# nfrasser/lasgun

Measured on NVIDIA B200. Metric: Mrays/s (primary+shadow), higher is better.
Workload: dtype f64

## Files before the change

### lasgun_b200/csrc/lgb_kernels.cu

```cuda
#include <math_constants.h>

#include <algorithm>

#include "lgb_math.cuh"

#ifndef LGB_SMEM_STACK
#define LGB_SMEM_STACK 0
#endif
#ifndef LGB_SMEM_TOP
#define LGB_SMEM_TOP 0
#endif
#define LGB_STK(i) ((i) * stride)
#ifndef LGB_WALK_PREFETCH
#define LGB_WALK_PREFETCH 0
#endif
#ifndef LGB_CP_STAGE
#define LGB_CP_STAGE 0
#endif
#ifndef LGB_WAVE_STREAM
#define LGB_WAVE_STREAM 1
#endif
#ifndef LGB_WALK_SPLIT
#define LGB_WALK_SPLIT 1
#endif
#ifndef LGB_WALK_SPLIT_SHADOW
#define LGB_WALK_SPLIT_SHADOW 0
#endif

namespace lgb {

#if LGB_WAVE_STREAM
template <class T> __device__ __forceinline__ void wst(T* p, T v) { __stcs(p, v); }
template <class T> __device__ __forceinline__ T wld(const T* p) { return __ldcs(p); }
#else
template <class T> __device__ __forceinline__ void wst(T* p, T v) { *p = v; }
template <class T> __device__ __forceinline__ T wld(const T* p) { return *p; }
#endif

struct RayF {
    float ox, oy, oz;
    float ix, iy, iz;
    float nx, ny, nz;
    float dx, dy, dz;
    float inv_dd, inv_len;
    float sx, sy, sz;
    float err;
    int kz;
    unsigned oct;
};

__device__ __forceinline__ float clamp_idir(float d) {
    const float v = 1.0f / d;
    return fabsf(v) > 1e30f ? copysignf(1e30f, v) : v;
}

__device__ __forceinline__ RayF make_rayf(const Ray64& r, float err_abs) {
    RayF f;
    f.ox = (float)r.o.x; f.oy = (float)r.o.y; f.oz = (float)r.o.z;
    f.dx = (float)r.d.x; f.dy = (float)r.d.y; f.dz = (float)r.d.z;
    f.oct = (signbit(r.d.x) ? 1u : 0u) | (signbit(r.d.y) ? 2u : 0u) | (signbit(r.d.z) ? 4u : 0u);
    f.ix = clamp_idir(f.dx); f.iy = clamp_idir(f.dy); f.iz = clamp_idir(f.dz);
    f.nx = -f.ox * f.ix; f.ny = -f.oy * f.iy; f.nz = -f.oz * f.iz;
    float dd = f.dx * f.dx + f.dy * f.dy + f.dz * f.dz;
    f.inv_dd = 1.0f / dd;
    f.inv_len = rsqrtf(dd);
    f.err = (dd > 1e-24f && dd < 1e24f) ? err_abs : CUDART_INF_F;
    f.kz = max_dimension_abs(r.d);
    const int kx = (f.kz + 1) % 3, ky = (kx + 1) % 3;
    float fdz = f.kz == 0 ? f.dx : (f.kz == 1 ? f.dy : f.dz);
    float fdx = kx == 0 ? f.dx : (kx == 1 ? f.dy : f.dz);
    float fdy = ky == 0 ? f.dx : (ky == 1 ? f.dy : f.dz);
    f.sz = 1.0f / fdz;
    f.sx = -fdx * f.sz;
    f.sy = -fdy * f.sz;
    return f;
}

__device__ __forceinline__ bool slab2(float lx, float ly, float lz, float hx, float hy, float hz, const RayF& f, float tbest_up, float& tnear_out) {
    float t1x = __fmaf_rn(lx, f.ix, f.nx), t2x = __fmaf_rn(hx, f.ix, f.nx);
    float t1y = __fmaf_rn(ly, f.iy, f.ny), t2y = __fmaf_rn(hy, f.iy, f.ny);
    float t1z = __fmaf_rn(lz, f.iz, f.nz), t2z = __fmaf_rn(hz, f.iz, f.nz);
    float tnear = fmaxf(fmaxf(fminf(t1x, t2x), fminf(t1y, t2y)), fminf(t1z, t2z));
    float tfar = fminf(fminf(fmaxf(t1x, t2x), fmaxf(t1y, t2y)), fmaxf(t1z, t2z));
    tnear_out = tnear;
    return tnear <= tfar * (1.0f + 9.5367431640625e-7f) && tfar > 0.0f && tnear <= tbest_up;
}
template <int OCT>
__device__ __forceinline__ bool slab_oct(float lx, float ly, float lz, float hx, float hy, float hz, const RayF& f, float tbest_up, float& tnear_out) {
    const float tnx = __fmaf_rn((OCT & 1) ? hx : lx, f.ix, f.nx), tfx = __fmaf_rn((OCT & 1) ? lx : hx, f.ix, f.nx);
    const float tny = __fmaf_rn((OCT & 2) ? hy : ly, f.iy, f.ny), tfy = __fmaf_rn((OCT & 2) ? ly : hy, f.iy, f.ny);
    const float tnz = __fmaf_rn((OCT & 4) ? hz : lz, f.iz, f.nz), tfz = __fmaf_rn((OCT & 4) ? lz : hz, f.iz, f.nz);
    const float tnear = fmaxf(fmaxf(tnx, tny), tnz);
    const float tfar = fminf(fminf(tfx, tfy), tfz) * (1.0f + 9.5367431640625e-7f);
    tnear_out = tnear;
    return fmaxf(tnear, 0.0f) <= fminf(tfar, tbest_up);
}
__device__ __forceinline__ float inflate_up(double t) { return __double2float_ru(t) * (1.0f + 9.5367431640625e-7f); }

struct Hit { double t; uint32_t ref; };

__device__ __forceinline__ DevCounters* ctr(const DevOut& O) {
    return reinterpret_cast<DevCounters*>(reinterpret_cast<char*>(O.counters) + (size_t)(1u + ((blockIdx.x + (threadIdx.x >> 5) * 17u) & (kCtrStripes - 1u))) * kCtrStride);
}
struct LocalCounters { unsigned int node_tests, filter[3], exact[3]; };

__device__ __forceinline__ uint32_t canonical_id(const DevScene& S, uint32_t ref) {
    const uint32_t type = ref >> 30, idx = ref & 0x3FFFFFFFu;
    if (type == LGB_PRIM_SPHERE) return S.sph_id[idx];
    if (type == LGB_PRIM_CUBOID) return S.cub_id[idx];
// ... 165 lines not shown
            if (tc + half + slack < 0.0f) continue;
            if (STATS) lc.exact[0]++;
            const double2 c01 = __ldg(reinterpret_cast<const double2*>(S.sph64 + 4 * (size_t)idx));
            const double2 c23 = __ldg(reinterpret_cast<const double2*>(S.sph64 + 4 * (size_t)idx + 2));
            double t; bool inside;
            if (sphere_exact(d3(c01.x, c01.y, c23.x), c23.y, ray, t, inside)) {
                const uint32_t ref = LGB_PRIM_REF(LGB_PRIM_SPHERE, idx);
                if (ANYHIT) { if (t < tmax) { best.t = t; best.ref = ref; return true; } }
                else if (accepts<INST>(S, f, world, best, t, ref, T.tied)) { best.t = t; best.ref = ref; best_tf = __double2float_ru(t); best_up = inflate_up(t); }
            }
        }
    } else {
        for (uint32_t i = 0; i < count; i++) {
            const uint32_t idx = first + i;
            const float4 lo = __ldg(&S.cub32[2 * idx]), hi = __ldg(&S.cub32[2 * idx + 1]);
            if (STATS) lc.filter[1]++;
            float tn;
            if (!slab2(lo.x, lo.y, lo.z, hi.x, hi.y, hi.z, f, CUDART_INF_F, tn)) continue;
            if (STATS) lc.exact[1]++;
            double mn[3], mx[3];
#pragma unroll
            for (int k = 0; k < 3; k++) { mn[k] = __ldg(&S.cub64[6 * (size_t)idx + k]); mx[k] = __ldg(&S.cub64[6 * (size_t)idx + 3 + k]); }
            double t; int ua, va;
            if (cuboid_exact(mn, mx, ray, t, ua, va)) {
                const uint32_t ref = LGB_PRIM_REF(LGB_PRIM_CUBOID, idx);
                if (ANYHIT) { if (t < tmax) { best.t = t; best.ref = ref; return true; } }
                else if (accepts<INST>(S, f, world, best, t, ref, T.tied)) { best.t = t; best.ref = ref; best_tf = __double2float_ru(t); best_up = inflate_up(t); }
            }
        }
    }
    return false;
}

template <bool STATS>
__device__ __forceinline__ bool prim_filter_rec(const RayF& f, float best_tf, uint32_t type, const float4 q0, const float4 q1, const float4 q2, LocalCounters& lc) {
    if (type == LGB_PRIM_SPHERE) {
        const float4 s = q0;
        if (STATS) lc.filter[0]++;
        const float lx = s.x - f.ox, ly = s.y - f.oy, lz = s.z - f.oz;
        const float bq = lx * f.dx + ly * f.dy + lz * f.dz;
        const float tc = bq * f.inv_dd;
        const float wx = __fmaf_rn(-tc, f.dx, lx), wy = __fmaf_rn(-tc, f.dy, ly), wz = __fmaf_rn(-tc, f.dz, lz);
        const float perp2 = wx * wx + wy * wy + wz * wz;
        const float rr = s.w + 2.0f * f.err;
        if (perp2 > rr * rr * (1.0f + 1e-6f)) return false;
        const float half = rr * f.inv_len;
        const float slack = fabsf(tc) * 2e-6f + 2.0f * f.err * f.inv_len;
        if (tc - half - slack > best_tf) return false;
        if (tc + half + slack < 0.0f) return false;
        return true;
    }
    if (type == LGB_PRIM_TRIANGLE) {
        if (STATS) lc.filter[2]++;
        return f.kz == 0 ? tri_filter<0>(q0, q1, q2, f, best_tf) : f.kz == 1 ? tri_filter<1>(q0, q1, q2, f, best_tf) : tri_filter<2>(q0, q1, q2, f, best_tf);
    }
    if (STATS) lc.filter[1]++;
    float tn;
    return slab2(q0.x, q0.y, q0.z, q1.x, q1.y, q1.z, f, CUDART_INF_F, tn);
}
__device__ __forceinline__ void prim_record(const DevScene& S, uint32_t type, uint32_t idx, float4& q0, float4& q1, float4& q2) {
    if (type == LGB_PRIM_SPHERE) q0 = __ldg(&S.sph32[idx]);
    else if (type == LGB_PRIM_TRIANGLE) { const float4* tp = S.tri + 3 * (size_t)idx; q0 = __ldg(tp); q1 = __ldg(tp + 1); q2 = __ldg(tp + 2); }
    else { q0 = __ldg(&S.cub32[2 * idx]); q1 = __ldg(&S.cub32[2 * idx + 1]); }
}
template <bool STATS>
__device__ __forceinline__ bool prim_filter(const DevScene& S, const RayF& f, float best_tf, uint32_t type, uint32_t idx, LocalCounters& lc) {
    float4 q0, q1 = make_float4(0.f, 0.f, 0.f, 0.f), q2 = q1;
    prim_record(S, type, idx, q0, q1, q2);
    return prim_filter_rec<STATS>(f, best_tf, type, q0, q1, q2, lc);
}
template <bool ANYHIT, bool STATS>
__device__ __forceinline__ bool prim_exact(const DevScene& S, const Ray64& world, const Ray64& ray, const RayF& f, Trav& T, uint32_t type, uint32_t idx, double tmax,
                                           LocalCounters& lc) {
    Hit& best = T.best;
    double t; bool ok;
    if (type == LGB_PRIM_SPHERE) {
        if (STATS) lc.exact[0]++;
        const double2 c01 = __ldg(reinterpret_cast<const double2*>(S.sph64 + 4 * (size_t)idx));
        const double2 c23 = __ldg(reinterpret_cast<const double2*>(S.sph64 + 4 * (size_t)idx + 2));
        bool inside;
        ok = sphere_exact(d3(c01.x, c01.y, c23.x), c23.y, ray, t, inside);
    } else if (type == LGB_PRIM_TRIANGLE) {
        if (STATS) lc.exact[2]++;
        const float4* tp = S.tri + 3 * (size_t)idx;
        const float4 q0 = __ldg(tp), q1 = __ldg(tp + 1), q2 = __ldg(tp + 2);
        double b0, b1, b2;
        ok = triangle_exact(d3(q0.x, q0.y, q0.z), d3(q1.x, q1.y, q1.z), d3(q2.x, q2.y, q2.z), ray, t, b0, b1, b2);
    } else {
        if (STATS) lc.exact[1]++;
        double mn[3], mx[3];
#pragma unroll
        for (int k = 0; k < 3; k++) { mn[k] = __ldg(&S.cub64[6 * (size_t)idx + k]); mx[k] = __ldg(&S.cub64[6 * (size_t)idx + 3 + k]); }
        int ua, va;
        ok = cuboid_exact(mn, mx, ray, t, ua, va);
    }
    if (!ok) return false;
    const uint32_t ref = LGB_PRIM_REF(type, idx);
    if (ANYHIT) { if (t < tmax) { best.t = t; best.ref = ref; return true; } return false; }
    if (accepts<false>(S, f, world, best, t, ref, T.tied)) { best.t = t; best.ref = ref; T.best_tf = __double2float_ru(t); T.best_up = inflate_up(t); }
    return false;
}

constexpr uint32_t kInstLeaf = kLeafBit | ((uint32_t)LGB_PRIM_INSTANCE << 29);
constexpr uint32_t kExitMarker = kInstLeaf | (31u << 24);
template <bool ANYHIT, bool STATS, bool REFILL, bool INST>
__device__ __forceinline__ bool trav_run(const DevScene& S, const Ray64& world, Ray64& ray, RayF& f, Trav& T, uint32_t* stack, float* tstack, double tmax,
                                         LocalCounters& lc, int refill_below, unsigned octw, const float4* top = nullptr, const int stride = 1) {
    Hit& best = T.best;
    float& best_tf = T.best_tf; float& best_up = T.best_up;
    uint32_t& cur = T.cur; int& sp = T.sp;
    for (;;) {
        switch (INST ? f.oct : octw) {
        case 0: node_loop<0, STATS, (!ANYHIT && LGB_TSTACK)>(S, f, best_up, cur, sp, stack, tstack, lc, top, stride); break;
        case 1: node_loop<1, STATS, (!ANYHIT && LGB_TSTACK)>(S, f, best_up, cur, sp, stack, tstack, lc, top, stride); break;
        case 2: node_loop<2, STATS, (!ANYHIT && LGB_TSTACK)>(S, f, best_up, cur, sp, stack, tstack, lc, top, stride); break;
        case 3: node_loop<3, STATS, (!ANYHIT && LGB_TSTACK)>(S, f, best_up, cur, sp, stack, tstack, lc, top, stride); break;
        case 4: node_loop<4, STATS, (!ANYHIT && LGB_TSTACK)>(S, f, best_up, cur, sp, stack, tstack, lc, top, stride); break;
        case 5: node_loop<5, STATS, (!ANYHIT && LGB_TSTACK)>(S, f, best_up, cur, sp, stack, tstack, lc, top, stride); break;
        case 6: node_loop<6, STATS, (!ANYHIT && LGB_TSTACK)>(S, f, best_up, cur, sp, stack, tstack, lc, top, stride); break;
        case 7: node_loop<7, STATS, (!ANYHIT && LGB_TSTACK)>(S, f, best_up, cur, sp, stack, tstack, lc, top, stride); break;
        default: node_loop<8, STATS, (!ANYHIT && LGB_TSTACK)>(S, f, best_up, cur, sp, stack, tstack, lc, top, stride); break;
        }
        if (cur == kDone) return true;
        {
            const uint32_t type = (cur >> 29) & 3u, count = ((cur >> 24) & 31u) + 1u, first = cur & kLeafFirstMask;
            if (INST && type == LGB_PRIM_INSTANCE) {
                if (count == 32u) {
                    T.space = first;
                    ray = ray_to_space(S, first, world);
                    f = make_rayf(ray, S.spaces[first].err_abs);
                } else {
                    if (count > 1u) { if (!ANYHIT && LGB_TSTACK) tstack[LGB_STK(sp)] = -CUDART_INF_F; stack[LGB_STK(sp)] = kInstLeaf | ((count - 2u) << 24) | (first + 1u); sp++; }
                    if (!ANYHIT && LGB_TSTACK) tstack[LGB_STK(sp)] = -CUDART_INF_F;
// ... 903 lines not shown
__device__ __noinline__ void setup_generic_slot(const DevScene* Sg, double ox, double oy, double oz, double dx, double dy, double dz, double t, uint32_t ref,
                                                double* ps_out, uint32_t* gate_out) {
    const DevScene& S = *Sg;
    Ray64 ray; ray.o = d3(ox, oy, oz); ray.d = d3(dx, dy, dz);
    ShadePoint P; uint32_t id;
    shade_point<false, false>(S, ray, t, ref, P, id);
    ps_out[0] = P.ps.x; ps_out[1] = P.ps.y; ps_out[2] = P.ps.z;
    *gate_out = light_gates(S, ray, P.ps, P.ng, dot(P.wo, P.ng), false);
}
#ifndef LGB_CPRIMARY_THREADS
#define LGB_CPRIMARY_THREADS 128
#endif
#ifndef LGB_CPRIMARY_BLOCKS
#define LGB_CPRIMARY_BLOCKS (1280 / LGB_CPRIMARY_THREADS)
#endif
template <bool STATS, bool SETUP = false>
__global__ void __launch_bounds__(LGB_CPRIMARY_THREADS, LGB_CPRIMARY_BLOCKS) k_cprimary(DevScene S, DevCamera C, DevWork W, DevOut O, DevWave V) {
    const uint64_t total = W.n_pixels * W.spp;
    const uint64_t g = (uint64_t)blockIdx.x * blockDim.x + threadIdx.x;
    const unsigned lane = threadIdx.x & 31u;
    LocalCounters lc = {};
    unsigned int hits = 0, primary = 0;
    bool valid = false;
    uint32_t x = 0, y = 0, s = 0;
    if (g < total) {
        const uint32_t p = fdiv((uint32_t)g, W.fd_spp);
        s = (uint32_t)g - p * W.spp;
        if (!slot_to_pixel(W, p, x, y)) { wst(&V.hit_t[g], (double)(CUDART_INF)); wst(&V.hit_ref[g], (uint32_t)(kSlotUnused)); }
        else valid = true;
    }
    const size_t cell = (size_t)(y >> W.cg_shift) * W.cg_nx + (size_t)(x >> W.cg_shift);
    uint32_t b = 0, e = 0;
    if (valid) { b = __ldg(W.cg_start + cell); e = __ldg(W.cg_start + cell + 1); }
#if LGB_CP_STAGE
    constexpr uint32_t kStage = 32;
    __shared__ uint2 s_ent[LGB_CPRIMARY_THREADS / 32][kStage];
    __shared__ float4 s_rec[LGB_CPRIMARY_THREADS / 32][kStage][3];
    const unsigned wid = threadIdx.x >> 5;
    uint32_t ns = 0;
    {
        const unsigned vmask = __ballot_sync(0xFFFFFFFFu, valid);
        if (vmask) {
            const int lead = __ffs(vmask) - 1;
            const unsigned long long cell0 = __shfl_sync(0xFFFFFFFFu, (unsigned long long)cell, lead);
            const uint32_t b0 = __shfl_sync(0xFFFFFFFFu, b, lead), e0 = __shfl_sync(0xFFFFFFFFu, e, lead);
            if (__all_sync(0xFFFFFFFFu, !valid || (unsigned long long)cell == cell0)) {
                ns = min(e0 - b0, kStage);
                if (lane < ns) {
                    const uint2 r = __ldg(W.cg_entries + b0 + lane);
                    float4 q0, q1 = make_float4(0.f, 0.f, 0.f, 0.f), q2 = q1;
                    prim_record(S, r.x >> 30, r.x & 0x3FFFFFFFu, q0, q1, q2);
                    s_ent[wid][lane] = r;
                    s_rec[wid][lane][0] = q0; s_rec[wid][lane][1] = q1; s_rec[wid][lane][2] = q2;
                }
                __syncwarp();
            }
        }
    }
#endif
    if (valid) {
        {
            const Ray64 world = camera_ray(C, W, x, y, s);
            Ray64 ray; RayF f; Trav T;
            enter_root<false>(S, world, ray, f, T, CUDART_INF);
            primary++;
            const float to_t = f.inv_len * (1.0f - 2e-6f);
            const bool sorted = e - b <= kGridSortMax;
#if LGB_WALK_SPLIT
            const uint32_t e2 = e + W.cg_n_large;
            for (uint32_t i = b;;) {
                uint32_t cand = 0xFFFFFFFFu;
                while (i < e2) {
                    const bool in_cell = i < e;
#if LGB_CP_STAGE
                    const uint32_t k = i - b;
                    const bool staged = k < ns;
                    const uint2 r = staged ? s_ent[wid][k] : __ldg(in_cell ? W.cg_entries + i : W.cg_large + (i - e));
                    i++;
                    if (__uint_as_float(r.y) * to_t > T.best_up) { if (!in_cell) i = e2; else if (sorted) i = e; continue; }
                    const uint32_t type = r.x >> 30;
                    float4 q0, q1 = make_float4(0.f, 0.f, 0.f, 0.f), q2 = q1;
                    if (staged) { q0 = s_rec[wid][k][0]; if (type != LGB_PRIM_SPHERE) { q1 = s_rec[wid][k][1]; q2 = s_rec[wid][k][2]; } }
                    else prim_record(S, type, r.x & 0x3FFFFFFFu, q0, q1, q2);
                    if (prim_filter_rec<STATS>(f, T.best_tf, type, q0, q1, q2, lc)) { cand = r.x; break; }
#else
                    const uint2 r = __ldg(in_cell ? W.cg_entries + i : W.cg_large + (i - e));
                    i++;
                    if (__uint_as_float(r.y) * to_t > T.best_up) { if (!in_cell) i = e2; else if (sorted) i = e; continue; }
                    if (prim_filter<STATS>(S, f, T.best_tf, r.x >> 30, r.x & 0x3FFFFFFFu, lc)) { cand = r.x; break; }
#endif
                }
                if (cand == 0xFFFFFFFFu) break;
                prim_exact<false, STATS>(S, world, ray, f, T, cand >> 30, cand & 0x3FFFFFFFu, CUDART_INF, lc);
            }
#else
#if LGB_WALK_PREFETCH
            uint2 nxt = b < e ? __ldg(W.cg_entries + b) : make_uint2(0u, 0u);
            for (uint32_t i = b; i < e; i++) {
                const uint2 r = nxt;
                if (i + 1 < e) nxt = __ldg(W.cg_entries + i + 1);
#else
            for (uint32_t i = b; i < e; i++) {
                const uint2 r = __ldg(W.cg_entries + i);
#endif
                if (__uint_as_float(r.y) * to_t > T.best_up) { if (sorted) break; else continue; }
                leaf_prims<false, STATS, false>(S, world, ray, f, T, r.x >> 30, 1u, r.x & 0x3FFFFFFFu, CUDART_INF, lc);
            }
            for (uint32_t i = 0; i < W.cg_n_large; i++) {
                const uint2 r = __ldg(W.cg_large + i);
                if (__uint_as_float(r.y) * to_t > T.best_up) break;
                leaf_prims<false, STATS, false>(S, world, ray, f, T, r.x >> 30, 1u, r.x & 0x3FFFFFFFu, CUDART_INF, lc);
            }
#endif
            const bool hit = T.best.ref != LGB_MISS;
            wst(&V.hit_t[g], (double)(hit ? T.best.t : CUDART_INF)); wst(&V.hit_ref[g], (uint32_t)(T.best.ref));
            hits += hit ? 1u : 0u;
            if (T.tied) { const uint32_t k = atomicAdd(V.tie_count, 1u); if (k < V.tie_cap) V.tie_list[k] = (uint32_t)g; }
            if (SETUP && hit) {
                const uint32_t ref = T.best.ref; const double t = T.best.t;
                if (S.specular && (material_flags(S, ref) & kMatSpecular)) { wst(&V.occl[g], (uint32_t)(0)); wst(&V.gate[g], (uint32_t)(0)); }
                else {
                    LeanSurf Ls;
                    lean_surface<true>(S, world, t, ref, 0u, Ls);
                    if (Ls.flags & kSfGeneric) setup_generic_slot(S.self, world.o.x, world.o.y, world.o.z, world.d.x, world.d.y, world.d.z, t, ref, V.ps + 3 * g, V.gate + g);
                    else {
                        const D3 ng = (Ls.flags & kSfNgFlip) ? -Ls.n : Ls.n;
                        const D3 ps = world.o + world.d * t + ng * (2.220446049250313e-16 * 65536.0);
                        wst(&V.ps[3 * g + 0], ps.x); wst(&V.ps[3 * g + 1], ps.y); wst(&V.ps[3 * g + 2], ps.z);
                        wst(&V.gate[g], (uint32_t)(light_gates(S, world, ps, ng, 1.0, true)));
                    }
                    wst(&V.sflags[g], (unsigned char)((unsigned char)Ls.flags));
                    wst(&V.occl[g], (uint32_t)(0));
                }
            }
        }
    }
    if (O.counters) {
        const unsigned long long v0 = __popc(__ballot_sync(0xFFFFFFFFu, primary != 0)), v1 = __popc(__ballot_sync(0xFFFFFFFFu, hits != 0));
        if (lane == 0) { atomicAdd(&ctr(O)->primary_rays, v0); atomicAdd(&ctr(O)->primary_hits, v1); }
        if (STATS) {
            for (int k = 0; k < 3; k++) {
                unsigned long long a = warp_sum(lc.filter[k]), b = warp_sum(lc.exact[k]);
                if (lane == 0) { atomicAdd(&ctr(O)->filter[k], a); atomicAdd(&ctr(O)->exact[k], b); atomicAdd(&ctr(O)->p_filter[k], a); atomicAdd(&ctr(O)->p_exact[k], b); }
            }
        }
    }
// ... 264 lines not shown
            const double* Lp = S.lights + 9 * (size_t)light;
            Ray64 world;
            world.o = d3(V.ps[3 * (size_t)g], V.ps[3 * (size_t)g + 1], V.ps[3 * (size_t)g + 2]);
            world.d = d3(Lp[0], Lp[1], Lp[2]) - world.o;
            Ray64 ray; RayF f; Trav T;
            enter_root<false>(S, world, ray, f, T, 1.0);
            bool hit = false;
            for (uint32_t k = 0; k < n && !hit; k++) {
                const uint2 e = __ldg(&list_in[(size_t)k * W.n_pixels + p]);
                hit = leaf_prims<true, STATS, false>(S, world, ray, f, T, (e.x >> 29) & 3u, 1u, e.x & kLeafFirstMask, 1.0, lc);
            }
            if (hit) { atomicOr(&V.occl[g], 1u << light); occluded++; }
            *slot = kEntryDone;
        }
    }
    if (O.counters) {
        unsigned long long v = warp_sum(occluded);
        if (lane == 0 && v) atomicAdd(&ctr(O)->shadow_occluded, v);
        if (STATS) {
            for (int k = 0; k < 3; k++) {
                unsigned long long a = warp_sum(lc.filter[k]), b = warp_sum(lc.exact[k]);
                if (lane == 0) { atomicAdd(&ctr(O)->filter[k], a); atomicAdd(&ctr(O)->exact[k], b); }
            }
        }
    }
}

#ifndef LGB_GSHADOW_THREADS
#define LGB_GSHADOW_THREADS 64
#endif
#ifndef LGB_GSHADOW_MIN_BLOCKS
#define LGB_GSHADOW_MIN_BLOCKS (1536 / LGB_GSHADOW_THREADS)
#endif
template <bool STATS>
__device__ __forceinline__ bool grid_blocked(const DevScene& S, D3 o, uint32_t l, LocalCounters& lc) {
    Ray64 world;
    world.o = o;
    const double* Lp = S.lights + 9 * (size_t)l;
    world.d = d3(Lp[0], Lp[1], Lp[2]) - world.o;
    const double ax = fabs(world.d.x), ay = fabs(world.d.y), az = fabs(world.d.z);
    const int a = ax >= ay ? (ax >= az ? 0 : 2) : (ay >= az ? 1 : 2);
    const double da = -(a == 0 ? world.d.x : a == 1 ? world.d.y : world.d.z);
    const double db = -(a == 0 ? world.d.y : a == 1 ? world.d.z : world.d.x), dc = -(a == 0 ? world.d.z : a == 1 ? world.d.x : world.d.y);
    if (da == 0.0) return false;
    const DevGrid* G = S.grids + l;
    const uint32_t res = __ldg(&G->res), n_large = __ldg(&G->n_large);
    const int face = 2 * a + (da < 0.0 ? 1 : 0);
    const double* map = G->map[face];
    const double inv = fast_rcp(fabs(da));
    const int cu = min(max((int)floor((db * inv - __ldg(map)) * __ldg(map + 1)), 0), (int)res - 1);
    const int cv = min(max((int)floor((dc * inv - __ldg(map + 2)) * __ldg(map + 3)), 0), (int)res - 1);
    const size_t cell = ((size_t)face * res + (size_t)cv) * res + (size_t)cu;
    const uint32_t* cs = G->cell_start;
    const uint32_t b = __ldg(cs + cell), e = __ldg(cs + cell + 1);
    Ray64 ray; RayF f; Trav T;
    enter_root<false>(S, world, ray, f, T, 1.0);
    const float dd = f.dx * f.dx + f.dy * f.dy + f.dz * f.dz;
    const float len_up = dd * f.inv_len * (1.0f + 1e-5f) + f.err;
    bool hit = false;
    const bool sorted = e - b <= kGridSortMax;
    const uint2* en = G->entries;
    const uint2* lg = G->large;
#if LGB_WALK_SPLIT_SHADOW
    const uint32_t e2 = e + n_large;
    for (uint32_t i = b;;) {
        uint32_t cand = 0xFFFFFFFFu;
        while (i < e2) {
            const bool in_cell = i < e;
            const uint2 r = __ldg(in_cell ? en + i : lg + (i - e));
            i++;
            if (__uint_as_float(r.y) > len_up) { if (!in_cell) i = e2; else if (sorted) i = e; continue; }
            if (prim_filter<STATS>(S, f, T.best_tf, r.x >> 30, r.x & 0x3FFFFFFFu, lc)) { cand = r.x; break; }
        }
        if (cand == 0xFFFFFFFFu) break;
        if (prim_exact<true, STATS>(S, world, ray, f, T, cand >> 30, cand & 0x3FFFFFFFu, 1.0, lc)) { hit = true; break; }
    }
#else
#if LGB_WALK_PREFETCH
    uint2 nxt = b < e ? __ldg(en + b) : make_uint2(0u, 0u);
    for (uint32_t i = b; i < e && !hit; i++) {
        const uint2 r = nxt;
        if (i + 1 < e) nxt = __ldg(en + i + 1);
#else
    for (uint32_t i = b; i < e && !hit; i++) {
        const uint2 r = __ldg(en + i);
#endif
        if (__uint_as_float(r.y) > len_up) { if (sorted) break; else continue; }
        hit = leaf_prims<true, STATS, false>(S, world, ray, f, T, r.x >> 30, 1u, r.x & 0x3FFFFFFFu, 1.0, lc);
    }
    for (uint32_t i = 0; i < n_large && !hit; i++) {
        const uint2 r = __ldg(lg + i);
        if (__uint_as_float(r.y) > len_up) break;
        hit = leaf_prims<true, STATS, false>(S, world, ray, f, T, r.x >> 30, 1u, r.x & 0x3FFFFFFFu, 1.0, lc);
    }
#endif
    return hit;
}

template <bool STATS, bool ALL_SHADOWS, bool SETUP = false>
__global__ void __launch_bounds__(LGB_GSHADOW_THREADS, LGB_GSHADOW_MIN_BLOCKS) k_gshadow(DevScene S, DevCamera C, DevWork W, DevOut O, DevWave V) {
    const uint64_t total = W.n_pixels * W.spp;
    const uint64_t g = (uint64_t)blockIdx.x * blockDim.x + threadIdx.x;
    const unsigned lane = threadIdx.x & 31u;
    LocalCounters lc = {};
    unsigned traced = 0, occluded = 0;
    if (g < total) {
        const uint32_t ref = wld(&V.hit_ref[g]);
        uint32_t mask = 0;
        D3 ps = d3(0, 0, 0);
        if (SETUP) {
            const double t = V.hit_t[g];
            Ray64 ray; uint32_t x, y, s;
            if (ref != LGB_MISS && ref != kSlotUnused && slot_ray<false>(C, W, g, ray, x, y, s)) {
                if (S.specular && (material_flags(S, ref) & kMatSpecular)) { V.occl[g] = 0; V.gate[g] = 0; }
                else {
                    LeanSurf Ls;
                    lean_surface<true>(S, ray, t, ref, 0u, Ls);
                    D3 ng; double wo_ng = 1.0;
                    if (Ls.flags & kSfGeneric) setup_generic(S, ray, t, ref, ps, ng, wo_ng);
                    else {
                        ng = (Ls.flags & kSfNgFlip) ? -Ls.n : Ls.n;
                        ps = ray.o + ray.d * t + ng * (2.220446049250313e-16 * 65536.0);
                    }
                    mask = light_gates(S, ray, ps, ng, wo_ng, !(Ls.flags & kSfGeneric));
                    V.gate[g] = mask; V.sflags[g] = (unsigned char)Ls.flags;
                    if (!mask) V.occl[g] = 0;
                }
            }
        } else {
            const uint32_t gate = ALL_SHADOWS ? (S.n_lights >= 32u ? 0xFFFFFFFFu : (1u << S.n_lights) - 1u) : wld(&V.gate[g]);
            ps = d3(wld(&V.ps[3 * g]), wld(&V.ps[3 * g + 1]), wld(&V.ps[3 * g + 2]));
            if (ref != LGB_MISS && ref != kSlotUnused) mask = gate;
        }
        if (mask) {
            uint32_t occl = 0;
            for (uint32_t l = 0; l < S.n_lights; l++) {
                if (!((mask >> l) & 1u)) continue;
                traced++;
                if (grid_blocked<STATS>(S, ps, l, lc)) { occl |= 1u << l; occluded++; }
            }
            wst(&V.occl[g], occl);
        }
    }
    if (O.counters) {
        const unsigned long long v0 = warp_sum(traced), v1 = warp_sum(occluded);
        if (lane == 0 && v0) {
            if (W.mode == 3) atomicAdd(&ctr(O)->secondary_rays, v0);
            else { atomicAdd(&ctr(O)->shadow_traced, v0); atomicAdd(&ctr(O)->shadow_occluded, v1); }
        }
        if (STATS) {
            for (int k = 0; k < 3; k++) {
                unsigned long long a = warp_sum(lc.filter[k]), b = warp_sum(lc.exact[k]);
                if (lane == 0) { atomicAdd(&ctr(O)->filter[k], a); atomicAdd(&ctr(O)->exact[k], b); }
            }
        }
    }
}

template <bool STATS, bool INST>
__global__ void __launch_bounds__(LGB_TRAV_THREADS, LGB_MIN_BLOCKS) k_shadow(DevScene S, DevWork W, DevOut O, DevWave V, uint32_t light, int which) {
    const unsigned total = V.queue_count[light * 3 + which];
    const uint32_t* q = V.queue + (size_t)(light * 3 + which) * V.queue_stride;
    const bool record = which == kQueueA && W.spp > 1;
    const double* L = S.lights + 9 * (size_t)light;
    const D3 lp = d3(L[0], L[1], L[2]);
    const unsigned lane = threadIdx.x & 31u;
    LocalCounters lc = {};
    unsigned int occluded = 0;
#if LGB_SMEM_STACK
    extern __shared__ uint32_t dyn_smem[];
    uint32_t* stack = dyn_smem + threadIdx.x;
    constexpr int kStride = LGB_TRAV_THREADS;
// ... 363 lines not shown
        rad[at] = output.x; rad[kRadStride + at] = output.y; rad[2 * kRadStride + at] = output.z;
        valid[threadIdx.x] = have ? 1 : 0;
    }
    __syncthreads();
    for (uint32_t j = threadIdx.x; j < 3u * ppb; j += blockDim.x) {
        const uint32_t ch = j >= 2u * ppb ? 2u : (j >= ppb ? 1u : 0u), q = j - ch * ppb, t0 = q * W.spp;
        if (!valid[t0]) continue;
        const double* r = rad + ch * kRadStride;
        double c = 0.0;
        for (uint32_t k = 0; k < W.spp; k++) c = c + r[t0 + k + ((t0 + k) >> 4)];
        c = c * (1.0 / (double)W.spp);
        bytes[3 * q + ch] = (unsigned char)round(fmin(fmax(c, 0.0), 1.0) * 255.0);
    }
    __syncthreads();
    if (threadIdx.x < ppb && valid[threadIdx.x * W.spp]) {
        const uint64_t p = ((uint64_t)blockIdx.x + W.block_off) * ppb + threadIdx.x;
        uint32_t px, py;
        slot_to_pixel(W, p, px, py);
        uchar4 o; o.x = bytes[3 * threadIdx.x]; o.y = bytes[3 * threadIdx.x + 1]; o.z = bytes[3 * threadIdx.x + 2]; o.w = 255;
        reinterpret_cast<uchar4*>(O.film)[W.compact_out ? W.compact_base + p : (uint64_t)py * W.w + px] = o;
    }
    }
}

#ifndef LGB_SURFACE_MIN_BLOCKS
#define LGB_SURFACE_MIN_BLOCKS 4
#endif
template <bool STATS>
__device__ __noinline__ D3 surface_generic(const DevScene& S, const DevShade& sh, const Ray64& ray, double t, uint32_t ref, LocalCounters& lc, unsigned& traced, unsigned& occluded) {
    ShadePoint P; uint32_t id;
    shade_point<false, false>(S, ray, t, ref, P, id);
    const uint32_t gate = light_gates(S, ray, P.ps, P.ng, dot(P.wo, P.ng), false);
    uint32_t occl = ~gate;
    for (uint32_t l = 0; l < S.n_lights; l++) {
        if (!((gate >> l) & 1u)) continue;
        traced++;
        if (grid_blocked<STATS>(S, P.ps, l, lc)) { occl |= 1u << l; occluded++; }
    }
    return shade_generic_plastic(S, sh, ray, t, ref, occl);
}
#ifndef LGB_SURFACE_THREADS
#define LGB_SURFACE_THREADS 256u
#endif
template <bool STATS>
__global__ void __launch_bounds__(256, LGB_SURFACE_MIN_BLOCKS) k_surface(DevScene S, DevCamera C, DevShade sh, DevWork W, DevOut O, DevWave V) {
    const double PI = 3.14159265358979323846264338327950288;
    __shared__ double rad[3 * kRadStride];
    __shared__ unsigned char valid[256];
    __shared__ unsigned char bytes[256 * 3];
    const unsigned lane = threadIdx.x & 31u;
    const uint32_t ppb = fdiv(blockDim.x, W.fd_spp);
    const uint32_t tp = fdiv(threadIdx.x, W.fd_spp), s = threadIdx.x - tp * W.spp;
    const uint64_t p = (uint64_t)blockIdx.x * ppb + tp;
    const bool mine = tp < ppb && p < W.n_pixels;
    const uint64_t g = p * W.spp + s;
    LocalCounters lc = {};
    unsigned traced = 0, occluded = 0;
    D3 output = d3(0, 0, 0);
    bool have = false, generic = false;
    uint32_t x = 0, y = 0;
    if (mine) {
        const uint32_t ref = V.hit_ref[g];
        const double t = V.hit_t[g];
        if (ref != kSlotUnused && slot_to_pixel(W, (uint32_t)p, x, y)) {
            const Ray64 ray = camera_ray(C, W, x, y, s);
            have = true;
            if (ref == LGB_MISS) output = background_of(sh, ray.d);
            else {
                LeanSurf Ls;
                lean_surface<true>(S, ray, t, ref, 0u, Ls);
                if (Ls.flags & kSfGeneric) generic = true;
                else {
                    const D3 ng = (Ls.flags & kSfNgFlip) ? -Ls.n : Ls.n;
                    const D3 ps = ray.o + ray.d * t + ng * (2.220446049250313e-16 * 65536.0);
                    uint32_t lit = light_gates(S, ray, ps, ng, 1.0, true);
                    for (uint32_t l = 0; l < S.n_lights; l++) {
                        if (!((lit >> l) & 1u)) continue;
                        traced++;
                        if (grid_blocked<STATS>(S, ps, l, lc)) { lit &= ~(1u << l); occluded++; }
                    }
                    output = lean_radiance(S, sh, ray, t, Ls, Ls.flags, lit);
                }
            }
        }
    }
    if (generic) {
        const Ray64 ray = camera_ray(C, W, x, y, s);
        output = surface_generic<STATS>(S, sh, ray, V.hit_t[g], V.hit_ref[g], lc, traced, occluded);
    }
    {
        const uint32_t at = threadIdx.x + (threadIdx.x >> 4);
        rad[at] = output.x; rad[kRadStride + at] = output.y; rad[2 * kRadStride + at] = output.z;
        valid[threadIdx.x] = have ? 1 : 0;
    }
    __syncthreads();
    for (uint32_t j = threadIdx.x; j < 3u * ppb; j += blockDim.x) {
        const uint32_t ch = j >= 2u * ppb ? 2u : (j >= ppb ? 1u : 0u), q = j - ch * ppb, t0 = q * W.spp;
        if (!valid[t0]) continue;
        const double* r = rad + ch * kRadStride;
        double c = 0.0;
        for (uint32_t k = 0; k < W.spp; k++) c = c + r[t0 + k + ((t0 + k) >> 4)];
        c = c * (1.0 / (double)W.spp);
        bytes[3 * q + ch] = (unsigned char)round(fmin(fmax(c, 0.0), 1.0) * 255.0);
    }
    __syncthreads();
    if (threadIdx.x < ppb && valid[threadIdx.x * W.spp]) {
        const uint64_t pp = (uint64_t)blockIdx.x * ppb + threadIdx.x;
        uint32_t px, py;
        slot_to_pixel(W, pp, px, py);
        uchar4 o; o.x = bytes[3 * threadIdx.x]; o.y = bytes[3 * threadIdx.x + 1]; o.z = bytes[3 * threadIdx.x + 2]; o.w = 255;
        reinterpret_cast<uchar4*>(O.film)[W.compact_out ? W.compact_base + pp : (uint64_t)py * W.w + px] = o;
    }
// ... 457 lines not shown
```

Before: 25660.

## Slim shadow grid walk: lazy ray setup, noinline exact test, pointer origin

Restructures the shadow-ray grid walk so the float ray record is built lazily. The slab and shear terms are now formed only when a cuboid or triangle filter runs, instead of going through the full enter_root setup. The double-precision exact test moves into a noinline shadow_exact function that rebuilds the ray from a pointer to the shading point and the light. This is meant to cut register pressure and live state in the hot shadow loop, at the cost of recomputing terms per candidate and a call overhead. It also removes dead prefetch, staging and split-walk variants, and simplifies prim_exact to return t so callers do their own acceptance.

```diff
diff --git a/lasgun_b200/csrc/lgb_kernels.cu b/lasgun_b200/csrc/lgb_kernels.cu
--- a/lasgun_b200/csrc/lgb_kernels.cu
+++ b/lasgun_b200/csrc/lgb_kernels.cu
@@ -11,22 +11,16 @@
 #define LGB_SMEM_TOP 0
 #endif
 #define LGB_STK(i) ((i) * stride)
-#ifndef LGB_WALK_PREFETCH
-#define LGB_WALK_PREFETCH 0
-#endif
-#ifndef LGB_CP_STAGE
-#define LGB_CP_STAGE 0
-#endif
 #ifndef LGB_WAVE_STREAM
 #define LGB_WAVE_STREAM 1
 #endif
-#ifndef LGB_WALK_SPLIT
-#define LGB_WALK_SPLIT 1
-#endif
-#ifndef LGB_WALK_SPLIT_SHADOW
-#define LGB_WALK_SPLIT_SHADOW 0
-#endif
-
+
+#ifndef LGB_GS_ONE_LOOP
+#define LGB_GS_ONE_LOOP 0
+#endif
+#ifndef LGB_GS_INLINE_SPHERE
+#define LGB_GS_INLINE_SPHERE 0
+#endif
 namespace lgb {
 
 #if LGB_WAVE_STREAM
@@ -75,6 +69,29 @@
     f.sy = -fdy * f.sz;
     return f;
 }
+__device__ __forceinline__ void rayf_lean(const Ray64& r, float err_abs, RayF& f) {
+    f.ox = (float)r.o.x; f.oy = (float)r.o.y; f.oz = (float)r.o.z;
+    f.dx = (float)r.d.x; f.dy = (float)r.d.y; f.dz = (float)r.d.z;
+    float dd = f.dx * f.dx + f.dy * f.dy + f.dz * f.dz;
+    f.inv_dd = 1.0f / dd;
+    f.inv_len = rsqrtf(dd);
+    f.err = (dd > 1e-24f && dd < 1e24f) ? err_abs : CUDART_INF_F;
+    f.kz = max_dimension_abs(r.d);
+}
+__device__ __forceinline__ void rayf_slab(RayF& f) {
+    f.ix = clamp_idir(f.dx); f.iy = clamp_idir(f.dy); f.iz = clamp_idir(f.dz);
+    f.nx = -f.ox * f.ix; f.ny = -f.oy * f.iy; f.nz = -f.oz * f.iz;
+}
+__device__ __forceinline__ void rayf_shear(RayF& f) {
+    const int kx = (f.kz + 1) % 3, ky = (kx + 1) % 3;
+    float fdz = f.kz == 0 ? f.dx : (f.kz == 1 ? f.dy : f.dz);
+    float fdx = kx == 0 ? f.dx : (kx == 1 ? f.dy : f.dz);
+    float fdy = ky == 0 ? f.dx : (ky == 1 ? f.dy : f.dz);
+    f.sz = 1.0f / fdz;
+    f.sx = -fdx * f.sz;
+    f.sy = -fdy * f.sz;
+}
+__device__ __forceinline__ void pin_dir(RayF& f) { asm volatile("" : "+f"(f.dx), "+f"(f.dy), "+f"(f.dz)); }
 
 __device__ __forceinline__ bool slab2(float lx, float ly, float lz, float hx, float hy, float hz, const RayF& f, float tbest_up, float& tnear_out) {
     float t1x = __fmaf_rn(lx, f.ix, f.nx), t2x = __fmaf_rn(hx, f.ix, f.nx);
@@ -306,7 +323,7 @@
     return false;
 }
 
-template <bool STATS>
+template <bool STATS, bool FORM_SLAB, bool FORM_SHEAR>
 __device__ __forceinline__ bool prim_filter_rec(const RayF& f, float best_tf, uint32_t type, const float4 q0, const float4 q1, const float4 q2, LocalCounters& lc) {
     if (type == LGB_PRIM_SPHERE) {
         const float4 s = q0;
@@ -326,53 +343,49 @@
     }
     if (type == LGB_PRIM_TRIANGLE) {
         if (STATS) lc.filter[2]++;
-        return f.kz == 0 ? tri_filter<0>(q0, q1, q2, f, best_tf) : f.kz == 1 ? tri_filter<1>(q0, q1, q2, f, best_tf) : tri_filter<2>(q0, q1, q2, f, best_tf);
+        RayF g = f;
+        if (FORM_SHEAR) { pin_dir(g); rayf_shear(g); }
+        return g.kz == 0 ? tri_filter<0>(q0, q1, q2, g, best_tf) : g.kz == 1 ? tri_filter<1>(q0, q1, q2, g, best_tf) : tri_filter<2>(q0, q1, q2, g, best_tf);
     }
     if (STATS) lc.filter[1]++;
+    RayF g = f;
+    if (FORM_SLAB) { pin_dir(g); rayf_slab(g); }
     float tn;
-    return slab2(q0.x, q0.y, q0.z, q1.x, q1.y, q1.z, f, CUDART_INF_F, tn);
+    return slab2(q0.x, q0.y, q0.z, q1.x, q1.y, q1.z, g, CUDART_INF_F, tn);
 }
 __device__ __forceinline__ void prim_record(const DevScene& S, uint32_t type, uint32_t idx, float4& q0, float4& q1, float4& q2) {
     if (type == LGB_PRIM_SPHERE) q0 = __ldg(&S.sph32[idx]);
     else if (type == LGB_PRIM_TRIANGLE) { const float4* tp = S.tri + 3 * (size_t)idx; q0 = __ldg(tp); q1 = __ldg(tp + 1); q2 = __ldg(tp + 2); }
     else { q0 = __ldg(&S.cub32[2 * idx]); q1 = __ldg(&S.cub32[2 * idx + 1]); }
 }
-template <bool STATS>
+template <bool STATS, bool FORM_SLAB, bool FORM_SHEAR>
 __device__ __forceinline__ bool prim_filter(const DevScene& S, const RayF& f, float best_tf, uint32_t type, uint32_t idx, LocalCounters& lc) {
     float4 q0, q1 = make_float4(0.f, 0.f, 0.f, 0.f), q2 = q1;
     prim_record(S, type, idx, q0, q1, q2);
-    return prim_filter_rec<STATS>(f, best_tf, type, q0, q1, q2, lc);
-}
-template <bool ANYHIT, bool STATS>
-__device__ __forceinline__ bool prim_exact(const DevScene& S, const Ray64& world, const Ray64& ray, const RayF& f, Trav& T, uint32_t type, uint32_t idx, double tmax,
-                                           LocalCounters& lc) {
-    Hit& best = T.best;
-    double t; bool ok;
+    return prim_filter_rec<STATS, FORM_SLAB, FORM_SHEAR>(f, best_tf, type, q0, q1, q2, lc);
+}
+template <bool STATS>
+__device__ __forceinline__ bool prim_exact(const DevScene& S, const Ray64& ray, uint32_t type, uint32_t idx, double& t, LocalCounters& lc) {
     if (type == LGB_PRIM_SPHERE) {
         if (STATS) lc.exact[0]++;
         const double2 c01 = __ldg(reinterpret_cast<const double2*>(S.sph64 + 4 * (size_t)idx));
         const double2 c23 = __ldg(reinterpret_cast<const double2*>(S.sph64 + 4 * (size_t)idx + 2));
         bool inside;
-        ok = sphere_exact(d3(c01.x, c01.y, c23.x), c23.y, ray, t, inside);
-    } else if (type == LGB_PRIM_TRIANGLE) {
+        return sphere_exact(d3(c01.x, c01.y, c23.x), c23.y, ray, t, inside);
+    }
+    if (type == LGB_PRIM_TRIANGLE) {
         if (STATS) lc.exact[2]++;
         const float4* tp = S.tri + 3 * (size_t)idx;
         const float4 q0 = __ldg(tp), q1 = __ldg(tp + 1), q2 = __ldg(tp + 2);
         double b0, b1, b2;
-        ok = triangle_exact(d3(q0.x, q0.y, q0.z), d3(q1.x, q1.y, q1.z), d3(q2.x, q2.y, q2.z), ray, t, b0, b1, b2);
-    } else {
-        if (STATS) lc.exact[1]++;
-        double mn[3], mx[3];
+        return triangle_exact(d3(q0.x, q0.y, q0.z), d3(q1.x, q1.y, q1.z), d3(q2.x, q2.y, q2.z), ray, t, b0, b1, b2);
+    }
+    if (STATS) lc.exact[1]++;
+    double mn[3], mx[3];
 #pragma unroll
-        for (int k = 0; k < 3; k++) { mn[k] = __ldg(&S.cub64[6 * (size_t)idx + k]); mx[k] = __ldg(&S.cub64[6 * (size_t)idx + 3 + k]); }
-        int ua, va;
-        ok = cuboid_exact(mn, mx, ray, t, ua, va);
-    }
-    if (!ok) return false;
-    const uint32_t ref = LGB_PRIM_REF(type, idx);
-    if (ANYHIT) { if (t < tmax) { best.t = t; best.ref = ref; return true; } return false; }
-    if (accepts<false>(S, f, world, best, t, ref, T.tied)) { best.t = t; best.ref = ref; T.best_tf = __double2float_ru(t); T.best_up = inflate_up(t); }
-    return false;
+    for (int k = 0; k < 3; k++) { mn[k] = __ldg(&S.cub64[6 * (size_t)idx + k]); mx[k] = __ldg(&S.cub64[6 * (size_t)idx + 3 + k]); }
+    int ua, va;
+    return cuboid_exact(mn, mx, ray, t, ua, va);
 }
 
 constexpr uint32_t kInstLeaf = kLeafBit | ((uint32_t)LGB_PRIM_INSTANCE << 29);
@@ -1342,32 +1355,6 @@
     const size_t cell = (size_t)(y >> W.cg_shift) * W.cg_nx + (size_t)(x >> W.cg_shift);
     uint32_t b = 0, e = 0;
     if (valid) { b = __ldg(W.cg_start + cell); e = __ldg(W.cg_start + cell + 1); }
-#if LGB_CP_STAGE
-    constexpr uint32_t kStage = 32;
-    __shared__ uint2 s_ent[LGB_CPRIMARY_THREADS / 32][kStage];
-    __shared__ float4 s_rec[LGB_CPRIMARY_THREADS / 32][kStage][3];
-    const unsigned wid = threadIdx.x >> 5;
-    uint32_t ns = 0;
-    {
-        const unsigned vmask = __ballot_sync(0xFFFFFFFFu, valid);
-        if (vmask) {
-            const int lead = __ffs(vmask) - 1;
-            const unsigned long long cell0 = __shfl_sync(0xFFFFFFFFu, (unsigned long long)cell, lead);
-            const uint32_t b0 = __shfl_sync(0xFFFFFFFFu, b, lead), e0 = __shfl_sync(0xFFFFFFFFu, e, lead);
-            if (__all_sync(0xFFFFFFFFu, !valid || (unsigned long long)cell == cell0)) {
-                ns = min(e0 - b0, kStage);
-                if (lane < ns) {
-                    const uint2 r = __ldg(W.cg_entries + b0 + lane);
-                    float4 q0, q1 = make_float4(0.f, 0.f, 0.f, 0.f), q2 = q1;
-                    prim_record(S, r.x >> 30, r.x & 0x3FFFFFFFu, q0, q1, q2);
-                    s_ent[wid][lane] = r;
-                    s_rec[wid][lane][0] = q0; s_rec[wid][lane][1] = q1; s_rec[wid][lane][2] = q2;
-                }
-                __syncwarp();
-            }
-        }
-    }
-#endif
     if (valid) {
         {
             const Ray64 world = camera_ray(C, W, x, y, s);
@@ -1376,52 +1363,24 @@
             primary++;
             const float to_t = f.inv_len * (1.0f - 2e-6f);
             const bool sorted = e - b <= kGridSortMax;
-#if LGB_WALK_SPLIT
             const uint32_t e2 = e + W.cg_n_large;
             for (uint32_t i = b;;) {
                 uint32_t cand = 0xFFFFFFFFu;
                 while (i < e2) {
                     const bool in_cell = i < e;
-#if LGB_CP_STAGE
-                    const uint32_t k = i - b;
-                    const bool staged = k < ns;
-                    const uint2 r = staged ? s_ent[wid][k] : __ldg(in_cell ? W.cg_entries + i : W.cg_large + (i - e));
-                    i++;
-                    if (__uint_as_float(r.y) * to_t > T.best_up) { if (!in_cell) i = e2; else if (sorted) i = e; continue; }
-                    const uint32_t type = r.x >> 30;
-                    float4 q0, q1 = make_float4(0.f, 0.f, 0.f, 0.f), q2 = q1;
-                    if (staged) { q0 = s_rec[wid][k][0]; if (type != LGB_PRIM_SPHERE) { q1 = s_rec[wid][k][1]; q2 = s_rec[wid][k][2]; } }
-                    else prim_record(S, type, r.x & 0x3FFFFFFFu, q0, q1, q2);
-                    if (prim_filter_rec<STATS>(f, T.best_tf, type, q0, q1, q2, lc)) { cand = r.x; break; }
-#else
                     const uint2 r = __ldg(in_cell ? W.cg_entries + i : W.cg_large + (i - e));
                     i++;
                     if (__uint_as_float(r.y) * to_t > T.best_up) { if (!in_cell) i = e2; else if (sorted) i = e; continue; }
-                    if (prim_filter<STATS>(S, f, T.best_tf, r.x >> 30, r.x & 0x3FFFFFFFu, lc)) { cand = r.x; break; }
-#endif
+                    if (prim_filter<STATS, false, false>(S, f, T.best_tf, r.x >> 30, r.x & 0x3FFFFFFFu, lc)) { cand = r.x; break; }
                 }
                 if (cand == 0xFFFFFFFFu) break;
-                prim_exact<false, STATS>(S, world, ray, f, T, cand >> 30, cand & 0x3FFFFFFFu, CUDART_INF, lc);
-            }
-#else
-#if LGB_WALK_PREFETCH
-            uint2 nxt = b < e ? __ldg(W.cg_entries + b) : make_uint2(0u, 0u);
-            for (uint32_t i = b; i < e; i++) {
-                const uint2 r = nxt;
-                if (i + 1 < e) nxt = __ldg(W.cg_entries + i + 1);
-#else
-            for (uint32_t i = b; i < e; i++) {
-                const uint2 r = __ldg(W.cg_entries + i);
-#endif
-                if (__uint_as_float(r.y) * to_t > T.best_up) { if (sorted) break; else continue; }
-                leaf_prims<false, STATS, false>(S, world, ray, f, T, r.x >> 30, 1u, r.x & 0x3FFFFFFFu, CUDART_INF, lc);
-            }
-            for (uint32_t i = 0; i < W.cg_n_large; i++) {
-                const uint2 r = __ldg(W.cg_large + i);
-                if (__uint_as_float(r.y) * to_t > T.best_up) break;
-                leaf_prims<false, STATS, false>(S, world, ray, f, T, r.x >> 30, 1u, r.x & 0x3FFFFFFFu, CUDART_INF, lc);
-            }
-#endif
+                const uint32_t type = cand >> 30, idx = cand & 0x3FFFFFFFu;
+                double t;
+                if (prim_exact<STATS>(S, ray, type, idx, t, lc)) {
+                    const uint32_t ref = LGB_PRIM_REF(type, idx);
+                    if (accepts<false>(S, f, world, T.best, t, ref, T.tied)) { T.best.t = t; T.best.ref = ref; T.best_tf = __double2float_ru(t); T.best_up = inflate_up(t); }
+                }
+            }
             const bool hit = T.best.ref != LGB_MISS;
             wst(&V.hit_t[g], (double)(hit ? T.best.t : CUDART_INF)); wst(&V.hit_ref[g], (uint32_t)(T.best.ref));
             hits += hit ? 1u : 0u;
@@ -1752,10 +1711,39 @@
 #ifndef LGB_GSHADOW_MIN_BLOCKS
 #define LGB_GSHADOW_MIN_BLOCKS (1536 / LGB_GSHADOW_THREADS)
 #endif
+__device__ __noinline__ bool shadow_exact(const DevScene* Sg, const double* po, uint32_t l, uint32_t ent) {
+    const DevScene& S = *Sg;
+    const double* Lp = S.lights + 9 * (size_t)l;
+    Ray64 ray;
+    ray.o = d3(po[0], po[1], po[2]);
+    ray.d = d3(Lp[0], Lp[1], Lp[2]) - ray.o;
+    LocalCounters lc;
+    double t;
+    return prim_exact<false>(S, ray, ent >> 30, ent & 0x3FFFFFFFu, t, lc) && t < 1.0;
+}
 template <bool STATS>
-__device__ __forceinline__ bool grid_blocked(const DevScene& S, D3 o, uint32_t l, LocalCounters& lc) {
+__device__ __forceinline__ bool shadow_entry(const DevScene& S, const double* po, uint32_t l, const RayF& f, uint32_t ent, LocalCounters& lc) {
+    const uint32_t type = ent >> 30;
+    if (!prim_filter<STATS, true, true>(S, f, 1.0f, type, ent & 0x3FFFFFFFu, lc)) return false;
+    if (STATS) lc.exact[type == LGB_PRIM_SPHERE ? 0 : type == LGB_PRIM_CUBOID ? 1 : 2]++;
+#if LGB_GS_INLINE_SPHERE
+    if (type == LGB_PRIM_SPHERE) {
+        double ox, oy, oz;
+        asm volatile("ld.f64 %0, [%3];\n\tld.f64 %1, [%3+8];\n\tld.f64 %2, [%3+16];" : "=d"(ox), "=d"(oy), "=d"(oz) : "l"(po));
+        const double* Lp = S.lights + 9 * (size_t)l;
+        Ray64 ray;
+        ray.o = d3(ox, oy, oz);
+        ray.d = d3(Lp[0], Lp[1], Lp[2]) - ray.o;
+        double t;
+        return prim_exact<false>(S, ray, type, ent & 0x3FFFFFFFu, t, lc) && t < 1.0;
+    }
+#endif
+    return shadow_exact(S.self, po, l, ent);
+}
+template <bool STATS>
+__device__ __forceinline__ bool grid_blocked(const DevScene& S, const double* po, uint32_t l, LocalCounters& lc) {
     Ray64 world;
-    world.o = o;
+    world.o = d3(po[0], po[1], po[2]);
     const double* Lp = S.lights + 9 * (size_t)l;
     world.d = d3(Lp[0], Lp[1], Lp[2]) - world.o;
     const double ax = fabs(world.d.x), ay = fabs(world.d.y), az = fabs(world.d.z);
@@ -1773,48 +1761,34 @@
     const size_t cell = ((size_t)face * res + (size_t)cv) * res + (size_t)cu;
     const uint32_t* cs = G->cell_start;
     const uint32_t b = __ldg(cs + cell), e = __ldg(cs + cell + 1);
-    Ray64 ray; RayF f; Trav T;
-    enter_root<false>(S, world, ray, f, T, 1.0);
+    RayF f;
+    rayf_lean(world, S.err_abs, f);
     const float dd = f.dx * f.dx + f.dy * f.dy + f.dz * f.dz;
     const float len_up = dd * f.inv_len * (1.0f + 1e-5f) + f.err;
-    bool hit = false;
     const bool sorted = e - b <= kGridSortMax;
     const uint2* en = G->entries;
     const uint2* lg = G->large;
-#if LGB_WALK_SPLIT_SHADOW
+#if LGB_GS_ONE_LOOP
     const uint32_t e2 = e + n_large;
-    for (uint32_t i = b;;) {
-        uint32_t cand = 0xFFFFFFFFu;
-        while (i < e2) {
-            const bool in_cell = i < e;
-            const uint2 r = __ldg(in_cell ? en + i : lg + (i - e));
-            i++;
-            if (__uint_as_float(r.y) > len_up) { if (!in_cell) i = e2; else if (sorted) i = e; continue; }
-            if (prim_filter<STATS>(S, f, T.best_tf, r.x >> 30, r.x & 0x3FFFFFFFu, lc)) { cand = r.x; break; }
-        }
-        if (cand == 0xFFFFFFFFu) break;
-        if (prim_exact<true, STATS>(S, world, ray, f, T, cand >> 30, cand & 0x3FFFFFFFu, 1.0, lc)) { hit = true; break; }
+    for (uint32_t i = b; i < e2; i++) {
+        const bool in_cell = i < e;
+        const uint2 r = __ldg(in_cell ? en + i : lg + (i - e));
+        if (__uint_as_float(r.y) > len_up) { if (!in_cell) break; if (sorted) i = e - 1; continue; }
+        if (shadow_entry<STATS>(S, po, l, f, r.x, lc)) return true;
     }
 #else
-#if LGB_WALK_PREFETCH
-    uint2 nxt = b < e ? __ldg(en + b) : make_uint2(0u, 0u);
-    for (uint32_t i = b; i < e && !hit; i++) {
-        const uint2 r = nxt;
-        if (i + 1 < e) nxt = __ldg(en + i + 1);
-#else
-    for (uint32_t i = b; i < e && !hit; i++) {
+    for (uint32_t i = b; i < e; i++) {
         const uint2 r = __ldg(en + i);
-#endif
         if (__uint_as_float(r.y) > len_up) { if (sorted) break; else continue; }
-        hit = leaf_prims<true, STATS, false>(S, world, ray, f, T, r.x >> 30, 1u, r.x & 0x3FFFFFFFu, 1.0, lc);
-    }
-    for (uint32_t i = 0; i < n_large && !hit; i++) {
+        if (shadow_entry<STATS>(S, po, l, f, r.x, lc)) return true;
+    }
+    for (uint32_t i = 0; i < n_large; i++) {
         const uint2 r = __ldg(lg + i);
         if (__uint_as_float(r.y) > len_up) break;
-        hit = leaf_prims<true, STATS, false>(S, world, ray, f, T, r.x >> 30, 1u, r.x & 0x3FFFFFFFu, 1.0, lc);
-    }
-#endif
-    return hit;
+        if (shadow_entry<STATS>(S, po, l, f, r.x, lc)) return true;
+    }
+#endif
+    return false;
 }
 
 template <bool STATS, bool ALL_SHADOWS, bool SETUP = false>
@@ -1827,8 +1801,10 @@
     if (g < total) {
         const uint32_t ref = wld(&V.hit_ref[g]);
         uint32_t mask = 0;
-        D3 ps = d3(0, 0, 0);
+        double ps_reg[3];
+        const double* po = V.ps + 3 * g;
         if (SETUP) {
+            D3 ps = d3(0, 0, 0);
             const double t = V.hit_t[g];
             Ray64 ray; uint32_t x, y, s;
             if (ref != LGB_MISS && ref != kSlotUnused && slot_ray<false>(C, W, g, ray, x, y, s)) {
@@ -1847,9 +1823,10 @@
                     if (!mask) V.occl[g] = 0;
                 }
             }
+            ps_reg[0] = ps.x; ps_reg[1] = ps.y; ps_reg[2] = ps.z;
+            po = ps_reg;
         } else {
             const uint32_t gate = ALL_SHADOWS ? (S.n_lights >= 32u ? 0xFFFFFFFFu : (1u << S.n_lights) - 1u) : wld(&V.gate[g]);
-            ps = d3(wld(&V.ps[3 * g]), wld(&V.ps[3 * g + 1]), wld(&V.ps[3 * g + 2]));
             if (ref != LGB_MISS && ref != kSlotUnused) mask = gate;
         }
         if (mask) {
@@ -1857,7 +1834,7 @@
             for (uint32_t l = 0; l < S.n_lights; l++) {
                 if (!((mask >> l) & 1u)) continue;
                 traced++;
-                if (grid_blocked<STATS>(S, ps, l, lc)) { occl |= 1u << l; occluded++; }
+                if (grid_blocked<STATS>(S, po, l, lc)) { occl |= 1u << l; occluded++; }
             }
             wst(&V.occl[g], occl);
         }
@@ -2287,10 +2264,11 @@
     shade_point<false, false>(S, ray, t, ref, P, id);
     const uint32_t gate = light_gates(S, ray, P.ps, P.ng, dot(P.wo, P.ng), false);
     uint32_t occl = ~gate;
+    const double po[3] = {P.ps.x, P.ps.y, P.ps.z};
     for (uint32_t l = 0; l < S.n_lights; l++) {
         if (!((gate >> l) & 1u)) continue;
         traced++;
-        if (grid_blocked<STATS>(S, P.ps, l, lc)) { occl |= 1u << l; occluded++; }
+        if (grid_blocked<STATS>(S, po, l, lc)) { occl |= 1u << l; occluded++; }
     }
     return shade_generic_plastic(S, sh, ray, t, ref, occl);
 }
@@ -2329,10 +2307,11 @@
                     const D3 ng = (Ls.flags & kSfNgFlip) ? -Ls.n : Ls.n;
                     const D3 ps = ray.o + ray.d * t + ng * (2.220446049250313e-16 * 65536.0);
                     uint32_t lit = light_gates(S, ray, ps, ng, 1.0, true);
+                    const double po[3] = {ps.x, ps.y, ps.z};
                     for (uint32_t l = 0; l < S.n_lights; l++) {
                         if (!((lit >> l) & 1u)) continue;
                         traced++;
-                        if (grid_blocked<STATS>(S, ps, l, lc)) { lit &= ~(1u << l); occluded++; }
+                        if (grid_blocked<STATS>(S, po, l, lc)) { lit &= ~(1u << l); occluded++; }
                     }
                     output = lean_radiance(S, sh, ray, t, Ls, Ls.flags, lit);
                 }
```

Result: faster. 26330 (median of 6 runs) (+2.6%).
